# ponimatkin/freepose

Hardware: AMD Instinct MI355X
Metric: proposals/sec (ViT-L feat + top-k + 576-pose render-compare) (higher is better)
Workload: dtype bf16

## Files before the change

freepose_amd/csrc/capi.hip:

```cpp
#include <stdarg.h>
#include <stdio.h>

#include "../../include/freepose_hip.h"
#include "tower_steps.h"
#include "pnp_core.h"
#include "video_eval_core.h"
#include "gt_info_core.h"
#include "lk_core.h"

static thread_local char g_err[512] = "";
void fp_set_error(const char* fmt, ...) {
    va_list ap;
    va_start(ap, fmt);
    vsnprintf(g_err, sizeof(g_err), fmt, ap);
    va_end(ap);
}
extern "C" const char* fp_last_error(void) { return g_err; }
extern "C" int fp_version(void) { return 100; }

#ifdef FP_LAB
static int g_opts[FP_OPT_COUNT] = {-1, -1, -1, -1, -1, -1, -1, -1, -1, -1, -1, -1};
int fp_opt_get(int key, int dflt) { return (key >= 0 && key < FP_OPT_COUNT && g_opts[key] >= 0) ? g_opts[key] : dflt; }
extern "C" int fp_lab_set_option(const char* name, int value) {
    FP_REQUIRE(name, "lab_set_option: null name");
// ... 544 lines not shown
    return fp_attention_hd_fwd((const bf16_t*)QKV, ldqkv, (bf16_t*)O, ldo, B, heads, head_dim, n_tok, npad, scale, (hipStream_t)stream);
}
extern "C" int fp_op_attention_causal(const void* QKV, int ldqkv, void* O, int ldo, int B, int heads, int head_dim, int n_tok, int npad,
                                      float scale, void* stream) {
    return fp_attention_causal_fwd((const bf16_t*)QKV, ldqkv, (bf16_t*)O, ldo, B, heads, head_dim, n_tok, npad, scale, (hipStream_t)stream);
}
extern "C" int fp_knn_l2(fp_ctx* ctx, const float* d_table, int N, int E, const float* d_queries, int Q, int k, int32_t* d_out_idx,
                         float* d_out_d2, void* stream) {
    FP_REQUIRE(ctx, "knn_l2: null context");
    FP_REQUIRE(N > 0 && Q > 0, "knn_l2: bad shape N=%d Q=%d", N, Q);
    float* ws = nullptr;
    FP_WS(ctx, "knn.d2", (size_t)Q * N * sizeof(float), ws);
    return fp_knn_l2_launch(d_table, N, E, d_queries, Q, k, ws, d_out_idx, d_out_d2, (hipStream_t)stream);
}
extern "C" int fp_op_im2col_norm(const void* img, void* A, int B, int H, int W, int ps, int KP, void* stream) {
    FP_REQUIRE(img && A && B > 0, "op_im2col_norm: null argument / empty batch");
    return fp_im2col_norm_ms((const bf16_t*)img, (bf16_t*)A, B, H, W, ps, KP, FP_IMAGENET_MEAN, FP_IMAGENET_SD, (hipStream_t)stream);
}
extern "C" int fp_op_layernorm(const void* X, void* Y, const void* g, const void* b, int rows, int D, float eps,
                               void* stream) {
    if (rows == 0) return FP_OK;
    FP_REQUIRE(X && Y && g && b, "op_layernorm: null argument");
    return fp_layernorm((const bf16_t*)X, (bf16_t*)Y, (const bf16_t*)g, (const bf16_t*)b, rows, D, eps, 0, 0, 0,
                        (hipStream_t)stream);
}
extern "C" int fp_op_layernorm_rows(const void* X, void* Y, const void* g, const void* b, int rows, int D, float eps, int rows_per_b,
                                    int in_stride_b, int in_off, int l2_normalize, void* stream) {
    FP_REQUIRE(rows >= 0 && D >= 0, "op_layernorm_rows: rows=%d, D=%d", rows, D);
    if (rows == 0 || D == 0) return FP_OK;
    FP_REQUIRE(X && Y && g && b, "op_layernorm_rows: null argument");
    FP_REQUIRE(rows_per_b <= 0 || (in_stride_b >= 0 && in_off >= 0), "op_layernorm_rows: in_stride_b=%d, in_off=%d (>= 0)", in_stride_b, in_off);
    return fp_layernorm((const bf16_t*)X, (bf16_t*)Y, (const bf16_t*)g, (const bf16_t*)b, rows, D, eps, rows_per_b, in_stride_b, in_off,
                        (hipStream_t)stream, l2_normalize != 0);
}
extern "C" int fp_op_posembed_aa(const void* src, void* dst, int G, int gh, int gw, int D, void* stream) {
    FP_REQUIRE(G >= 0 && gh >= 0 && gw >= 0 && D >= 0, "op_posembed_aa: G=%d, gh=%d, gw=%d, D=%d", G, gh, gw, D);
    if (gh == 0 || gw == 0 || D == 0) return FP_OK;
    FP_REQUIRE(src && dst, "op_posembed_aa: null argument");
    return fp_posembed_aa((const bf16_t*)src, (bf16_t*)dst, G, gh, gw, D, (hipStream_t)stream);
}
extern "C" int fp_op_token_init(void* X, const void* cls, const void* pos0, const void* reg, int nreg, int B, int n_tok, int npad, int D,
                                void* stream) {
    FP_REQUIRE(B >= 0 && B <= 65535 && D >= 0, "op_token_init: B=%d (0..65535), D=%d", B, D);
    FP_REQUIRE(nreg >= 0 && n_tok >= 1 + nreg && npad >= n_tok, "op_token_init: nreg=%d, n_tok=%d, npad=%d (1 + nreg <= n_tok <= npad)", nreg, n_tok,
               npad);
    if (B == 0 || D == 0) return FP_OK;
    FP_REQUIRE(X && cls && pos0 && (reg || nreg == 0), "op_token_init: null argument");
    FP_REQUIRE((long long)(1 + nreg + npad - n_tok) * D <= INT32_MAX, "op_token_init: %d rows of %d elements", 1 + nreg + npad - n_tok, D);
    return fp_token_init((bf16_t*)X, (const bf16_t*)cls, (const bf16_t*)pos0, (const bf16_t*)reg, nreg, B, n_tok, npad, D, (hipStream_t)stream);
}
extern "C" int fp_op_row_stats(const void* X, int rows, int D, float eps, void* d_rec, float* d_rstd, void* stream) {
    FP_REQUIRE(rows >= 0 && D >= 0, "op_row_stats: rows=%d, D=%d", rows, D);
    if (rows == 0) return FP_OK;
    FP_REQUIRE(X && d_rec && d_rstd, "op_row_stats: null argument");
    FP_REQUIRE(D > 0, "op_row_stats: D=%d", D);
    return fp_row_stats((const bf16_t*)X, (uint4*)d_rec, d_rstd, rows, D, eps, (hipStream_t)stream);
}
extern "C" int fp_op_stats_finalize(const void* part, int rows, int D, float eps, int part_ld, void* d_rec, float* d_rstd, void* stream) {
    FP_REQUIRE(rows >= 0 && D >= 0, "op_stats_finalize: rows=%d, D=%d", rows, D);
    if (rows == 0) return FP_OK;
    FP_REQUIRE(part && d_rec && d_rstd, "op_stats_finalize: null argument");
    FP_REQUIRE(D > 0 && (part_ld == 0 || part_ld >= rows), "op_stats_finalize: D=%d, part_ld=%d (0 or >= rows=%d)", D, part_ld, rows);
    return fp_stats_finalize((const float2*)part, (uint4*)d_rec, d_rstd, rows, D, eps, (hipStream_t)stream, part_ld);
}
extern "C" int fp_op_ln_fold(const void* W, const void* gamma, const void* beta, const void* bias, int N, int K, int n_scaled, float row_scale,
                             void* Wf, void* d_cb, void* stream) {
    FP_REQUIRE(N >= 0 && K >= 0, "op_ln_fold: N=%d, K=%d", N, K);
    if (N == 0) return FP_OK;
    FP_REQUIRE(K > 0 && n_scaled >= 0 && n_scaled <= N, "op_ln_fold: K=%d, n_scaled=%d outside [0, N=%d]", K, n_scaled, N);
    return fp_ln_fold((const bf16_t*)W, (const bf16_t*)gamma, (const bf16_t*)beta, (const bf16_t*)bias, (bf16_t*)Wf, (uint4*)d_cb, N, K, n_scaled,
                      row_scale, (hipStream_t)stream);
}
extern "C" int fp_op_transpose(const void* src, void* dst, int rows, int cols, void* stream) {
    FP_REQUIRE(rows >= 0 && cols >= 0, "op_transpose: rows=%d, cols=%d", rows, cols);
    if (rows == 0 || cols == 0) return FP_OK;
    FP_REQUIRE(src && dst, "op_transpose: null argument");
    return fp_transpose_bf16((const bf16_t*)src, (bf16_t*)dst, rows, cols, (hipStream_t)stream);
}

struct FpTimer { hipEvent_t a, b; };
extern "C" int fp_timer_create(void** out) {
    FP_REQUIRE(out, "timer_create: null");
    FpTimer* t = new FpTimer();
    FP_HIP(hipEventCreate(&t->a));
    FP_HIP(hipEventCreate(&t->b));
    *out = t;
    return FP_OK;
}
extern "C" int fp_timer_start(void* t, void* s) { FP_HIP(hipEventRecord(((FpTimer*)t)->a, (hipStream_t)s)); return FP_OK; }
extern "C" int fp_timer_stop(void* t, void* s) { FP_HIP(hipEventRecord(((FpTimer*)t)->b, (hipStream_t)s)); return FP_OK; }
extern "C" int fp_timer_elapsed_ms(void* t, float* ms) {
    FP_HIP(hipEventSynchronize(((FpTimer*)t)->b));
    FP_HIP(hipEventElapsedTime(ms, ((FpTimer*)t)->a, ((FpTimer*)t)->b));
    return FP_OK;
}
extern "C" int fp_timer_destroy(void* t) {
    if (!t) return FP_OK;
    (void)hipEventDestroy(((FpTimer*)t)->a);
    (void)hipEventDestroy(((FpTimer*)t)->b);
    delete (FpTimer*)t;
    return FP_OK;
}

#define FP_LK_MAX_QUERIES (1 << 20)
static int lk_check_sizes(const char* what, int T, int H, int W, int levels, int radius) {
    FP_REQUIRE(T >= 1 && T <= 65535, "%s: T=%d frames (1..65535)", what, T);
    FP_REQUIRE(H >= 1 && W >= 1 && H <= FP_LK_MAX_SIDE && W <= FP_LK_MAX_SIDE, "%s: %d x %d frames (1..%d per side)", what, H, W, FP_LK_MAX_SIDE);
    FP_REQUIRE((long long)T * H * W <= (1ll << 30), "%s: T * H * W = %lld pixels (at most 2^30 per call)", what, (long long)T * H * W);
    FP_REQUIRE(radius >= 1 && radius <= FP_LK_MAX_RADIUS, "%s: radius=%d (1..%d)", what, radius, FP_LK_MAX_RADIUS);
    FP_REQUIRE(levels >= 1 && levels <= FP_LK_MAX_LEVELS, "%s: levels=%d (1..%d)", what, levels, FP_LK_MAX_LEVELS);
    return FP_OK;
}

extern "C" int fp_lk_pyramid(fp_ctx* ctx, const uint8_t* d_frames, int T, int H, int W, int levels, int radius, float* d_pyramid, void* stream) {
    FP_REQUIRE(ctx && d_frames && d_pyramid, "lk_pyramid: null argument");
    if (int rc = lk_check_sizes("lk_pyramid", T, H, W, levels, radius)) return rc;
    LkPyramid P;
    lk_pyramid_layout(T, H, W, levels, radius, P);
    return fp_lk_pyramid_launch(d_frames, P, d_pyramid, (hipStream_t)stream);
}

extern "C" int fp_lk_track(fp_ctx* ctx, const float* d_pyramid, int T, int H, int W, int levels, const float* d_queries, int N, int radius,
                           int iters, float fb_thresh, float min_eig, float max_residual, float* d_tracks, uint8_t* d_vis, float* d_diag,
                           void* stream) {
    if (int rc = lk_check_sizes("lk_track", T, H, W, levels, radius)) return rc;
    FP_REQUIRE(N >= 0 && N <= FP_LK_MAX_QUERIES, "lk_track: N=%d queries (0..2^20)", N);
    FP_REQUIRE(ctx && d_pyramid && (N == 0 || (d_queries && d_tracks && d_vis && d_diag)), "lk_track: null argument");
    FP_REQUIRE(iters >= 1 && iters <= FP_LK_MAX_ITERS, "lk_track: iters=%d (1..%d)", iters, FP_LK_MAX_ITERS);
    LkPyramid P;
    lk_pyramid_layout(T, H, W, levels, radius, P);
    double* state = nullptr;
    if (N > 0) FP_WS(ctx, "lk_state", (size_t)T * N * 2 * sizeof(double), state);
    return fp_lk_track_launch(P, d_pyramid, d_queries, N, radius, iters, fb_thresh, min_eig, max_residual, state, d_tracks, d_vis, d_diag,
                              (hipStream_t)stream);
}
```

freepose_amd/csrc/tower_steps.h:

```cpp
#pragma once
#include <stdio.h>
#include <string.h>

#include <cmath>

#include "internal.h"

struct GemmStep {
    FpGemmArgs g{};
    int epi;
    GemmStep(const bf16_t* X, int ldx, const bf16_t* W, int K, bf16_t* C, int ldc, const bf16_t* bias, int M, int N, bool gelu = false)
        : epi(gelu ? FP_EPI_BIAS_GELU : FP_EPI_BIAS) {
        g.X = X; g.ldx = ldx; g.W = W; g.ldw = K; g.C = C; g.ldc = ldc; g.bias = bias;
        g.M = M; g.N = N; g.K = K;
    }
    GemmStep& residual(const bf16_t* gamma, const bf16_t* resid, int ldr, float2* stat_part = nullptr) {
        g.gamma = gamma; g.resid = resid; g.ldr = ldr; g.stat_part = stat_part;
        epi = stat_part ? FP_EPI_LS_RES_STATS : FP_EPI_BIAS_LS_RES;
        return *this;
    }
    GemmStep& transposed_v(int npad, int heads) {
        g.ldc = 8; g.npad = npad; g.heads = heads;
        epi = FP_EPI_VT;
        return *this;
    }
    GemmStep& patch_embed(const bf16_t* pos, int P, int npad, int tok_off) {
        g.pos = pos; g.P = P; g.npad = npad; g.tok_off = tok_off;
        epi = FP_EPI_PATCH;
        return *this;
    }
    int run(fp_ctx* ctx, hipStream_t s) { return ctx->gemm(g, epi, s); }
};

struct LnStats {
    uint4* stat; float* rstd; float2* part;
    int M, D; float eps;
    bool pending = false;
    int ready(const bf16_t* rows, int N, hipStream_t s) {
        pending = !rows && fp_gemm_fuses_ln_part(M, N);
        if (rows) return fp_row_stats(rows, stat, rstd, M, D, eps, s);
        return pending ? FP_OK : fp_stats_finalize(part, stat, rstd, M, D, eps, s);
    }
    int attach(GemmStep& t, const uint4* cfrag) {
        FP_REQUIRE(t.epi == FP_EPI_BIAS || t.epi == FP_EPI_BIAS_GELU || t.epi == FP_EPI_VT, "ln attach: epilogue %d has no LN-folded form", t.epi);
        t.g.ln_mfrag = stat; t.g.ln_rstd = rstd; t.g.ln_cfrag = cfrag;
        t.epi = t.epi == FP_EPI_BIAS ? FP_EPI_LN_BIAS : (t.epi == FP_EPI_BIAS_GELU ? FP_EPI_LN_GELU : FP_EPI_LN_VT);
        if (pending) { t.g.ln_part = part; t.g.ln_part_ld = M; t.g.ln_part_nb = D / 64; t.g.ln_eps = eps; t.g.ln_inv_d = 1.0f / (float)D; }
        pending = false;
        return FP_OK;
    }
};

enum TowerCls { TOWER_GEMM = 0, TOWER_ATTN = 1, TOWER_OTHER = 2 };
struct TowerProf {
    bool on = false;
    struct EvPair { hipEvent_t a, b; int cls; };
    std::vector<EvPair> ev_pool;
    size_t ev_used = 0;
    double gemm_flops = 0;
    long gemm_launches = 0;
    void count(double flops, int launches) { if (on) { gemm_flops += flops; gemm_launches += launches; } }
};
struct ProfScope {
    TowerProf* p; hipStream_t s; size_t slot;
    ProfScope(TowerProf* p_, hipStream_t s_, TowerCls cls) : p(p_), s(s_), slot((size_t)-1) {
        if (!p || !p->on) return;
        if (p->ev_used == p->ev_pool.size()) {
            TowerProf::EvPair e{};
            if (hipEventCreate(&e.a) != hipSuccess || hipEventCreate(&e.b) != hipSuccess) return;
            p->ev_pool.push_back(e);
        }
        slot = p->ev_used++;
        p->ev_pool[slot].cls = cls;
        (void)hipEventRecord(p->ev_pool[slot].a, s);
    }
    ~ProfScope() {
        if (slot != (size_t)-1) (void)hipEventRecord(p->ev_pool[slot].b, s);
    }
};

struct TowerBlockW {
    const bf16_t *n1w = nullptr, *n1b = nullptr, *qkvw = nullptr, *qkvb = nullptr, *projw = nullptr,
                 *projb = nullptr, *ls1 = nullptr, *n2w = nullptr, *n2b = nullptr, *fc1w = nullptr, *fc1b = nullptr,
                 *fc2w = nullptr, *fc2b = nullptr, *ls2 = nullptr;
    bool complete() const { return n1w && n1b && qkvw && qkvb && projw && projb && n2w && n2b && fc1w && fc1b && fc2w && fc2b; }
};
struct TowerRun {
    fp_ctx* ctx; TowerProf* prof; hipStream_t s;
    int B, n_tok, npad, D, mlp_dim;
    float eps;
    bf16_t *R, *T, *AO, *H1;
    const bf16_t* ones;
    int M() const { return B * npad; }
    void count(double flops_per_row, int launches) const { if (prof) prof->count((double)B * n_tok * flops_per_row, launches); }
};
struct TowerEmbedW {
    int patch = 0, KP = 0, n_reg = 0;
    const float *mean = nullptr, *sd = nullptr;
    bf16_t* pe_w = nullptr;
    const bf16_t *pe_b = nullptr, *cls = nullptr, *pos = nullptr, *reg = nullptr;
};
inline int fp_tower_embed(const TowerRun& t, const TowerEmbedW& e, const bf16_t* pos_patch, const bf16_t* img, int H, int W, bf16_t* A0, bf16_t* X) {
    const int P = (H / e.patch) * (W / e.patch);
    int rc;
    {
        ProfScope ps(t.prof, t.s, TOWER_OTHER);
        if ((rc = fp_im2col_norm_ms(img, A0, t.B, H, W, e.patch, e.KP, e.mean, e.sd, t.s))) return rc;
        if ((rc = fp_token_init(X, e.cls, e.pos, e.reg, e.n_reg, t.B, t.n_tok, t.npad, t.D, t.s))) return rc;
    }
    ProfScope ps(t.prof, t.s, TOWER_GEMM);
    GemmStep pe(A0, e.KP, e.pe_w, e.KP, X, t.D, e.pe_b, t.B * P, t.D);
    if ((rc = pe.patch_embed(pos_patch, P, t.npad, 1 + e.n_reg).run(t.ctx, t.s))) return rc;
    if (t.prof) t.prof->count(2.0 * t.B * P * (3.0 * e.patch * e.patch) * t.D, 1);
    return FP_OK;
}
inline int fp_tower_out_proj(const TowerRun& t, const TowerBlockW& w, float2* stat_part) {
    ProfScope ps(t.prof, t.s, TOWER_GEMM);
    GemmStep proj(t.AO, t.D, w.projw, t.D, t.R, t.D, w.projb, t.M(), t.D);
    if (int rc = proj.residual(w.ls1 ? w.ls1 : t.ones, t.R, t.D, stat_part).run(t.ctx, t.s)) return rc;
    t.count(2.0 * t.D * t.D, 1);
    return FP_OK;
}
inline int fp_tower_mlp(const TowerRun& t, const TowerBlockW& w, LnStats* st, const bf16_t* fc1w, const uint4* fc1_cb, float2* stat_part) {
    const int D = t.D, M = t.M(), N = t.mlp_dim;
    int rc;
    {
        ProfScope ps(t.prof, t.s, TOWER_OTHER);
        if ((rc = st ? st->ready(nullptr, N, t.s) : fp_layernorm(t.R, t.T, w.n2w, w.n2b, M, D, t.eps, 0, 0, 0, t.s))) return rc;
    }
    ProfScope ps(t.prof, t.s, TOWER_GEMM);
    GemmStep fc1(st ? t.R : t.T, D, st ? fc1w : w.fc1w, D, t.H1, N, w.fc1b, M, N, true);
    if (st && (rc = st->attach(fc1, fc1_cb))) return rc;
    if ((rc = fc1.run(t.ctx, t.s))) return rc;
    if ((rc = GemmStep(t.H1, N, w.fc2w, N, t.R, D, w.fc2b, M, D).residual(w.ls2 ? w.ls2 : t.ones, t.R, D, stat_part).run(t.ctx, t.s))) return rc;
    t.count(4.0 * D * N, 2);
    return FP_OK;
}

inline bool fp_weight_numel(const char* who, const char* name, size_t numel, size_t want) {
    if (numel != want) fp_set_error("%s: %s has %zu elements, expected %zu", who, name, numel, want);
    return numel == want;
}
struct WeightEnt { const char* n; const bf16_t** slot; size_t numel; };
template <size_t N>
inline int fp_set_named_weight(const char* who, const char* name, const char* rest, const WeightEnt (&tab)[N], const bf16_t* p, size_t numel) {
    for (const WeightEnt& e : tab)
        if (!strcmp(rest, e.n)) {
            if (!fp_weight_numel(who, name, numel, e.numel)) return -1;
            *e.slot = p;
            return 1;
        }
    return 0;
}
inline int fp_tower_set_patch_weight(const char* who, const char* name, const bf16_t* p, size_t numel, const TowerEmbedW& e, size_t D, hipStream_t s) {
    const size_t K = (size_t)3 * e.patch * e.patch;
    if (!fp_weight_numel(who, name, numel, D * K)) return FP_ERR_INVALID;
    FP_HIP(hipMemcpy2DAsync(e.pe_w, (size_t)e.KP * 2, p, K * 2, K * 2, D, hipMemcpyDeviceToDevice, s));
    return FP_OK;
}

// ... 84 lines not shown
```

freepose_amd/csrc/vit.hip:

```cpp
#include <stdio.h>

#include "../../include/freepose_hip.h"
#include "tower_steps.h"

struct fp_vit {
    fp_ctx* ctx = nullptr;
    fp_vit_arch a{};
    TowerEmbedW emb;
    const bf16_t *normw = nullptr, *normb = nullptr;
    bf16_t* ones = nullptr;
    std::vector<TowerBlockW> blk;
    struct VitFold { bf16_t *qkvw = nullptr, *fc1w = nullptr; uint4 *qkv_cb = nullptr, *fc1_cb = nullptr; };
    std::vector<VitFold> fold;
    int folded_upto = 0;
    hipEvent_t fold_ev = nullptr;
    hipStream_t fold_stream = nullptr;
    bool refold = false;
    std::map<std::pair<int, int>, bf16_t*> pos_cache;
    TowerProf prof;
};

extern "C" int fp_vit_create(fp_ctx* ctx, const fp_vit_arch* arch, fp_vit** out) {
    FP_REQUIRE(ctx && arch && out, "vit_create: null argument");
    FP_REQUIRE(arch->dim % 64 == 0 && arch->heads * 64 == arch->dim, "vit_create: dim=%d heads=%d (head dim must be 64)",
               arch->dim, arch->heads);
    FP_REQUIRE(arch->mlp_dim % 64 == 0 && arch->depth > 0 && arch->patch > 0, "vit_create: bad arch");
    fp_vit* v = new fp_vit();
    v->ctx = ctx;
    v->a = *arch;
    v->blk.resize(arch->depth);
    v->fold.resize(arch->depth);
    v->emb.patch = arch->patch; v->emb.n_reg = arch->n_reg; v->emb.mean = FP_IMAGENET_MEAN; v->emb.sd = FP_IMAGENET_SD;
    v->emb.KP = cdiv(3 * arch->patch * arch->patch, 64) * 64;
    if (hipMalloc((void**)&v->emb.pe_w, (size_t)arch->dim * v->emb.KP * 2) != hipSuccess ||
        hipMalloc((void**)&v->ones, (size_t)arch->dim * 2) != hipSuccess) {
        fp_set_error("vit_create: hipMalloc failed");
        delete v;
        return FP_ERR_HIP;
    }
    FP_HIP(hipMemset(v->emb.pe_w, 0, (size_t)arch->dim * v->emb.KP * 2));
    std::vector<bf16_t> one(arch->dim, f2bf(1.0f));
    FP_HIP(hipMemcpy(v->ones, one.data(), (size_t)arch->dim * 2, hipMemcpyHostToDevice));
    *out = v;
    return FP_OK;
}
extern "C" int fp_vit_destroy(fp_vit* v) {
    if (!v) return FP_OK;
    if (v->emb.pe_w) (void)hipFree(v->emb.pe_w);
    if (v->ones) (void)hipFree(v->ones);
    for (auto& kv : v->pos_cache) (void)hipFree(kv.second);
    for (auto& f : v->fold) {
        if (f.qkvw) (void)hipFree(f.qkvw);
        if (f.fc1w) (void)hipFree(f.fc1w);
        if (f.qkv_cb) (void)hipFree(f.qkv_cb);
        if (f.fc1_cb) (void)hipFree(f.fc1_cb);
    }
    for (auto& p : v->prof.ev_pool) { (void)hipEventDestroy(p.a); (void)hipEventDestroy(p.b); }
    if (v->fold_ev) (void)hipEventDestroy(v->fold_ev);
    delete v;
    return FP_OK;
}

extern "C" int fp_vit_set_weight(fp_vit* v, const char* name, const void* d, size_t numel, void* stream) {
    FP_REQUIRE(v && name && d, "vit_set_weight: null argument");
    const fp_vit_arch& a = v->a;
    const bf16_t* p = (const bf16_t*)d;
    const size_t D = a.dim;
    if (v->folded_upto > 0) v->refold = true;
    v->folded_upto = 0;
    std::string s(name);
    if (s == "pos_embed") {
        if (!fp_weight_numel("vit_set_weight", name, numel, (size_t)(1 + a.pos_grid * a.pos_grid) * D)) return FP_ERR_INVALID;
        v->emb.pos = p;
        for (auto& kv : v->pos_cache) (void)hipFree(kv.second);
        v->pos_cache.clear();
        return FP_OK;
    }
    if (s == "mask_token") return FP_OK;
    if (s == "patch_embed.proj.weight") return fp_tower_set_patch_weight("vit_set_weight", name, p, numel, v->emb, D, (hipStream_t)stream);
    const WeightEnt top[] = {{"cls_token", &v->emb.cls, D}, {"register_tokens", &v->emb.reg, (size_t)a.n_reg * D}, {"patch_embed.proj.bias", &v->emb.pe_b, D},
                             {"norm.weight", &v->normw, D}, {"norm.bias", &v->normb, D}};
    if (const int hit = fp_set_named_weight("vit_set_weight", name, name, top, p, numel)) return hit > 0 ? FP_OK : FP_ERR_INVALID;
    int bi = -1;
    char rest[64] = {0};
    if (sscanf(name, "blocks.%d.%63s", &bi, rest) == 2 && bi >= 0 && bi < a.depth) {
        TowerBlockW& w = v->blk[bi];
        const size_t M = a.mlp_dim;
        const WeightEnt tab[] = {
            {"norm1.weight", &w.n1w, D}, {"norm1.bias", &w.n1b, D},
            {"attn.qkv.weight", &w.qkvw, 3 * D * D}, {"attn.qkv.bias", &w.qkvb, 3 * D},
            {"attn.proj.weight", &w.projw, D * D}, {"attn.proj.bias", &w.projb, D},
            {"ls1.gamma", &w.ls1, D}, {"norm2.weight", &w.n2w, D}, {"norm2.bias", &w.n2b, D},
            {"mlp.fc1.weight", &w.fc1w, M * D}, {"mlp.fc1.bias", &w.fc1b, M},
            {"mlp.fc2.weight", &w.fc2w, D * M}, {"mlp.fc2.bias", &w.fc2b, D}, {"ls2.gamma", &w.ls2, D}};
        if (const int hit = fp_set_named_weight("vit_set_weight", name, rest, tab, p, numel)) return hit > 0 ? FP_OK : FP_ERR_INVALID;
    }
    fp_set_error("vit_set_weight: unknown tensor name '%s'", name);
    return FP_ERR_INVALID;
}

static int vit_pos(fp_vit* v, int gh, int gw, hipStream_t s, const bf16_t** out) {
    const fp_vit_arch& a = v->a;
    if (gh == a.pos_grid && gw == a.pos_grid) { *out = v->emb.pos + a.dim; return FP_OK; }
    auto key = std::make_pair(gh, gw);
    auto it = v->pos_cache.find(key);
    if (it == v->pos_cache.end()) {
        bf16_t* buf = nullptr;
        FP_HIP(hipMalloc((void**)&buf, (size_t)gh * gw * a.dim * 2));
        int rc = fp_posembed_aa(v->emb.pos + a.dim, buf, a.pos_grid, gh, gw, a.dim, s);
        if (rc) { (void)hipFree(buf); return rc; }
        it = v->pos_cache.emplace(key, buf).first;
    }
    *out = it->second;
    return FP_OK;
}

static int vit_fold(fp_vit* v, int first, int L, hipStream_t s) {
    const fp_vit_arch& a = v->a;
    const size_t D = a.dim, Mm = a.mlp_dim;
    for (int i = first; i < L; ++i) {
        const TowerBlockW& w = v->blk[i];
        fp_vit::VitFold& f = v->fold[i];
        if (!f.qkvw) FP_HIP(hipMalloc((void**)&f.qkvw, 3 * D * D * 2));
        if (!f.qkv_cb) FP_HIP(hipMalloc((void**)&f.qkv_cb, 3 * D * sizeof(uint4)));
        if (!f.fc1w) FP_HIP(hipMalloc((void**)&f.fc1w, Mm * D * 2));
        if (!f.fc1_cb) FP_HIP(hipMalloc((void**)&f.fc1_cb, Mm * sizeof(uint4)));
        int rc;
        if ((rc = fp_ln_fold(w.qkvw, w.n1w, w.n1b, w.qkvb, f.qkvw, f.qkv_cb, (int)(3 * D), (int)D, (int)D, FP_ATTN_QSCALE, s))) return rc;
        if ((rc = fp_ln_fold(w.fc1w, w.n2w, w.n2b, w.fc1b, f.fc1w, f.fc1_cb, (int)Mm, (int)D, 0, 1.0f, s))) return rc;
    }
    return FP_OK;
}

extern "C" double fp_vit_flops(const fp_vit* v, int B, int H, int W, int layer) {
    const fp_vit_arch& a = v->a;
    const double P = (double)(H / a.patch) * (W / a.patch), N = P + 1 + a.n_reg, D = a.dim;
    const int L = std::min(layer, a.depth);
    const double mlp_ratio = (double)a.mlp_dim / a.dim;
    const double per_block = (8.0 + 4.0 * mlp_ratio) * N * D * D + 4.0 * N * N * D;
    return B * (L * per_block + 2.0 * P * (3.0 * a.patch * a.patch) * D);
}

extern "C" int fp_vit_forward(fp_vit* v, const void* d_images, int B, int H, int W, int layer, int feature_type,
                              void* d_out, void* stream) {
    FP_REQUIRE(v && d_images && d_out, "vit_forward: null argument");
    const fp_vit_arch& a = v->a;
    hipStream_t s = (hipStream_t)stream;
    fp_ctx* ctx = v->ctx;
    FP_REQUIRE(B > 0 && H % a.patch == 0 && W % a.patch == 0, "vit_forward: B=%d H=%d W=%d (patch %d)", B, H, W, a.patch);
    FP_REQUIRE(feature_type >= 0 && feature_type <= 3, "vit_forward: feature_type %d", feature_type);
    FP_REQUIRE(v->emb.cls && v->emb.pos && v->emb.pe_b && v->normw && v->normb && (a.n_reg == 0 || v->emb.reg),
               "vit_forward: embedding / final-norm weights not set");
    const int L = (layer >= 1 && layer <= a.depth) ? layer : a.depth;
    for (int i = 0; i < L; ++i) {
        FP_REQUIRE(v->blk[i].complete(), "vit_forward: weights of block %d not set", i);
    }
    const int D = a.dim, gh = H / a.patch, gw = W / a.patch, P = gh * gw;
    const int n_tok = P + 1 + a.n_reg;
    const int npad = cdiv(n_tok, 16) * 16;
    const size_t M = (size_t)B * npad;
    FP_REQUIRE(M * (size_t)a.mlp_dim * 2 < 0xffffffffull, "vit_forward: batch too large for 32-bit tile offsets (B=%d)", B);
    const int Mi = (int)M;

    bf16_t *A0, *X, *Y, *QK, *Vt, *AO, *H1;
    int rc;
    const bool lnf = ctx->opt_ln_fused != 0 && D % 64 == 0;
    LnStats st{nullptr, nullptr, nullptr, Mi, D, a.ln_eps};
    if (lnf) {
        if (v->fold_ev && s != v->fold_stream) FP_HIP(hipStreamWaitEvent(s, v->fold_ev, 0));
        if (v->folded_upto < L) {
            if (v->refold) {
                FP_HIP(hipDeviceSynchronize());
                v->refold = false;
            }
            if ((rc = vit_fold(v, v->folded_upto, L, s))) return rc;
            if (!v->fold_ev) FP_HIP(hipEventCreateWithFlags(&v->fold_ev, hipEventDisableTiming));
            FP_HIP(hipEventRecord(v->fold_ev, s));
            v->fold_stream = s;
            v->folded_upto = L;
        }
        FP_WS(ctx, "vit.ln_stat", M * sizeof(uint4), st.stat);
        FP_WS(ctx, "vit.ln_rstd", M * sizeof(float), st.rstd);
        FP_WS(ctx, "vit.ln_part", M * (size_t)(D / 64) * sizeof(float2), st.part);
    }
    FP_WS(ctx, "vit.im2col", (size_t)B * P * v->emb.KP * 2, A0);
    FP_WS(ctx, "vit.x", M * D * 2, X);
    FP_WS(ctx, "vit.y", M * D * 2, Y);
    FP_WS(ctx, "vit.qk", M * 2 * D * 2, QK);
    FP_WS(ctx, "vit.vt", M * D * 2 + 256, Vt);
    FP_WS(ctx, "vit.ao", M * D * 2, AO);
    FP_WS(ctx, "vit.h1", M * (size_t)a.mlp_dim * 2, H1);

    const bf16_t* pos_patch;
    if ((rc = vit_pos(v, gh, gw, s, &pos_patch))) return rc;

    const TowerRun t{ctx, &v->prof, s, B, n_tok, npad, D, a.mlp_dim, a.ln_eps, X, Y, AO, H1, v->ones};
    if ((rc = fp_tower_embed(t, v->emb, pos_patch, (const bf16_t*)d_images, H, W, A0, X))) return rc;
    const bf16_t* in = lnf ? X : Y;
    for (int i = 0; i < L; ++i) {
        const TowerBlockW& w = v->blk[i];
        const fp_vit::VitFold& f = v->fold[i];
        {
            ProfScope ps(&v->prof, s, TOWER_OTHER);
            if ((rc = lnf ? st.ready(i == 0 ? X : nullptr, 2 * D, s) : fp_layernorm(X, Y, w.n1w, w.n1b, Mi, D, a.ln_eps, 0, 0, 0, s))) return rc;
        }
        {
            ProfScope ps(&v->prof, s, TOWER_GEMM);
            const bf16_t* qkvw = lnf ? f.qkvw : w.qkvw;
            GemmStep qk(in, D, qkvw, D, QK, 2 * D, w.qkvb, Mi, 2 * D), vt(in, D, qkvw + (size_t)2 * D * D, D, Vt, 8, w.qkvb + 2 * D, Mi, D);
            vt.transposed_v(npad, a.heads);
            if (lnf && ((rc = st.attach(qk, f.qkv_cb)) || (rc = st.attach(vt, f.qkv_cb + 2 * D)))) return rc;
            if ((rc = qk.run(ctx, s))) return rc;
            if ((rc = vt.run(ctx, s))) return rc;
            t.count(2.0 * 3.0 * D * D, 2);
        }
        {
            ProfScope ps(&v->prof, s, TOWER_ATTN);
            if ((rc = fp_attention_fwd(QK, 2 * D, Vt, AO, D, B, a.heads, n_tok, npad, lnf, s))) return rc;
        }
        if ((rc = fp_tower_out_proj(t, w, st.part))) return rc;
        if ((rc = fp_tower_mlp(t, w, lnf ? &st : nullptr, f.fc1w, f.fc1_cb, i + 1 < L ? st.part : nullptr))) return rc;
    }
    {
        ProfScope ps(&v->prof, s, TOWER_OTHER);
        const int rows_per_b = feature_type == 0 ? 1 : (feature_type == 1 ? a.n_reg : P);
        const int off = feature_type == 0 ? 0 : (feature_type == 1 ? 1 : 1 + a.n_reg);
        if (rows_per_b > 0)
            if ((rc = fp_layernorm(X, (bf16_t*)d_out, v->normw, v->normb, B * rows_per_b, D, a.ln_eps, rows_per_b, npad,
                                   off, s, feature_type == 3)))
                return rc;
    }
    return FP_OK;
}

extern "C" int fp_vit_profile(fp_vit* v, int enable) {
    FP_REQUIRE(v, "vit_profile: null");
    TowerProf& p = v->prof;
    p.on = enable != 0;
    p.ev_used = 0;
    p.gemm_flops = 0;
    p.gemm_launches = 0;
    return FP_OK;
}
extern "C" int fp_vit_profile_read(fp_vit* v, float* g, float* at, float* o, double* fl) {
    FP_REQUIRE(v, "vit_profile_read: null");
    TowerProf& p = v->prof;
    float acc[3] = {0.f, 0.f, 0.f};
    for (size_t i = 0; i < p.ev_used; ++i) {
        FP_HIP(hipEventSynchronize(p.ev_pool[i].b));
        float ms = 0.f;
        FP_HIP(hipEventElapsedTime(&ms, p.ev_pool[i].a, p.ev_pool[i].b));
        acc[p.ev_pool[i].cls] += ms;
    }
    if (g) *g = acc[TOWER_GEMM];
    if (at) *at = acc[TOWER_ATTN];
    if (o) *o = acc[TOWER_OTHER];
    if (fl) *fl = p.gemm_flops;
    return FP_OK;
}
extern "C" long fp_vit_profile_gemm_launches(const fp_vit* v) { return v ? v->prof.gemm_launches : 0; }
```

freepose_amd/csrc/vit_misc.hip:

```cpp
#include "internal.h"
#include "dot64.h"
#include "gemm_bf16.h"

namespace {

__global__ void im2col_norm_kernel(const bf16_t* __restrict__ img, bf16_t* __restrict__ A, int B, int H,
                                   int W, int ps, int KP, float m0, float m1, float m2, float s0, float s1,
                                   float s2) {
    const int gw = W / ps, gh = H / ps, P = gw * gh;
    const int K = 3 * ps * ps;
    const int chunks = KP / 8;
    const long total = (long)B * P * chunks;
    for (long idx = blockIdx.x * (long)blockDim.x + threadIdx.x; idx < total;
         idx += (long)gridDim.x * blockDim.x) {
        const int ch = (int)(idx % chunks);
        const long row = idx / chunks;
        const int b = (int)(row / P), pp = (int)(row % P);
        const int py = pp / gw, px = pp % gw;
        uint32_t w[4];
#pragma unroll
        for (int e = 0; e < 8; e += 2) {
            float v[2];
#pragma unroll
            for (int u = 0; u < 2; ++u) {
                const int k = ch * 8 + e + u;
                float val = 0.f;
                if (k < K) {
                    const int c = k / (ps * ps), rem = k % (ps * ps);
                    const int dy = rem / ps, dx = rem % ps;
                    const float x = bf2f(img[(((size_t)b * 3 + c) * H + (py * ps + dy)) * W + px * ps + dx]);
                    const float mean = c == 0 ? m0 : (c == 1 ? m1 : m2);
                    const float sd = c == 0 ? s0 : (c == 1 ? s1 : s2);
                    val = rbf(rbf(x - mean) / sd);
                }
                v[u] = val;
            }
            w[e / 2] = pack_bf2(v[0], v[1]);
        }
        *(uint4*)(A + (size_t)row * KP + ch * 8) = make_uint4(w[0], w[1], w[2], w[3]);
    }
}

__global__ void token_init_kernel(bf16_t* __restrict__ X, const bf16_t* __restrict__ cls,
                                  const bf16_t* __restrict__ pos0, const bf16_t* __restrict__ reg, int nreg,
                                  int n_tok, int npad, int D) {
    const int b = blockIdx.y;
    const int nrows = 1 + nreg + (npad - n_tok);
    for (int i = blockIdx.x * blockDim.x + threadIdx.x; i < nrows * D; i += gridDim.x * blockDim.x) {
        const int r = i / D, c = i % D;
        int row;
        bf16_t v;
        if (r == 0) { row = 0; v = f2bf(bf2f(cls[c]) + bf2f(pos0[c])); }
        else if (r <= nreg) { row = r; v = reg[(r - 1) * D + c]; }
        else { row = n_tok + (r - 1 - nreg); v = 0; }
        X[((size_t)b * npad + row) * D + c] = v;
    }
}

template <int MAXC, int L2 = 0>
__global__ __launch_bounds__(256) void layernorm_kernel(const bf16_t* __restrict__ X, bf16_t* __restrict__ Y,
                                                        const bf16_t* __restrict__ gamma,
                                                        const bf16_t* __restrict__ beta, int rows, int D,
                                                        float eps, int rows_per_b, int in_stride_b, int in_off) {
    const int lane = threadIdx.x & 63;
    const int wave = (blockIdx.x * blockDim.x + threadIdx.x) >> 6;
    const int nwave = (gridDim.x * blockDim.x) >> 6;
    const int nch = D / 8;
    for (int r = wave; r < rows; r += nwave) {
        const size_t ir = (size_t)(r / rows_per_b) * in_stride_b + in_off + (r % rows_per_b);
        const bf16_t* xr = X + ir * D;
        uint4 xw[MAXC];
        float v[MAXC][8];
        d64_load<MAXC>(xw, xr, 0, D, lane);
        d64_unpack(xw, v);
        float sum = 0.f;
#pragma unroll
        for (int c = 0; c < MAXC; ++c)
            if (lane + 64 * c < nch) {
#pragma unroll
                for (int e = 0; e < 8; ++e) sum += v[c][e];
            }
        const float mean = wave_sum(sum) / (float)D;
        float sq = 0.f;
#pragma unroll
        for (int c = 0; c < MAXC; ++c)
            if (lane + 64 * c < nch) {
#pragma unroll
                for (int e = 0; e < 8; ++e) { const float d = v[c][e] - mean; sq += d * d; }
            }
        const float rstd = rsqrtf(wave_sum(sq) / (float)D + eps);
        bf16_t* yr = Y + (size_t)r * D;
        uint4 keep[MAXC];
        float acc = 0.f;
#pragma unroll
        for (int c = 0; c < MAXC; ++c) {
            const int ch = lane + 64 * c;
            if (ch < nch) {
                const uint4 g = *(const uint4*)(gamma + ch * 8), bb = *(const uint4*)(beta + ch * 8);
                const uint32_t gw[4] = {g.x, g.y, g.z, g.w}, bw[4] = {bb.x, bb.y, bb.z, bb.w};
                uint32_t o[4];
#pragma unroll
                for (int e = 0; e < 4; ++e) {
                    const float a = (v[c][2 * e] - mean) * rstd * lo_bf(gw[e]) + lo_bf(bw[e]);
                    const float b = (v[c][2 * e + 1] - mean) * rstd * hi_bf(gw[e]) + hi_bf(bw[e]);
                    o[e] = pack_bf2(a, b);
                }
                if (L2) {
                    keep[c] = make_uint4(o[0], o[1], o[2], o[3]);
                    acc = d64_sumsq(keep[c], acc);
                } else {
                    *(uint4*)(yr + ch * 8) = make_uint4(o[0], o[1], o[2], o[3]);
                }
            }
        }
        if (L2) d64_norm_store<MAXC>(keep, d64_row_norm(wave_sum(acc)), yr, D, lane);
    }
}

__device__ __forceinline__ float cubic_aa(float x) {
    const float a = -0.5f;
    x = fabsf(x);
    if (x < 1.f) return ((a + 2.f) * x - (a + 3.f)) * x * x + 1.f;
// ... 203 lines not shown
            }
        const float sigma = __fsqrt_rn(wave_sum(sq) / (float)D + eps);
        if (lane == 0) { mfrag[r] = ln_row_record(mean, sigma); rstd_out[r] = __builtin_amdgcn_rcpf(sigma); }

    }
}

__global__ __launch_bounds__(256) void stats_finalize_kernel(const float2* __restrict__ part, uint4* __restrict__ mfrag,
                                                             float* __restrict__ rstd_out, int rows, int nb, float inv_d, float eps, int part_ld) {
    const int r = blockIdx.x * blockDim.x + threadIdx.x;
    if (r >= rows) return;
    uint4 rec;
    float rstd;
    fp_ln_finalize_row(part, (size_t)part_ld, nb, r, inv_d, eps, rec, rstd);
    mfrag[r] = rec;
    rstd_out[r] = rstd;
}

__global__ __launch_bounds__(256) void ln_fold_kernel(const bf16_t* __restrict__ W, const bf16_t* __restrict__ gamma,
                                                      const bf16_t* __restrict__ beta, const bf16_t* __restrict__ bias,
                                                      bf16_t* __restrict__ Wf, uint4* __restrict__ cfrag, int N, int K, int n_scaled,
                                                      float row_scale) {
    const int lane = threadIdx.x & 63;
    const int n = (blockIdx.x * blockDim.x + threadIdx.x) >> 6;
    if (n >= N) return;
    const float rs = n < n_scaled ? row_scale : 1.0f;
    float cs = 0.f, wb = 0.f;
    for (int k = lane * 8; k < K; k += 512) {
        const uint4 w = *(const uint4*)(W + (size_t)n * K + k), g = *(const uint4*)(gamma + k), b = *(const uint4*)(beta + k);
        const uint32_t ww[4] = {w.x, w.y, w.z, w.w}, gw[4] = {g.x, g.y, g.z, g.w}, bw[4] = {b.x, b.y, b.z, b.w};
        uint32_t o[4];
#pragma unroll
        for (int e = 0; e < 4; ++e) {
            const float f0 = rbf(lo_bf(ww[e]) * lo_bf(gw[e]) * rs), f1 = rbf(hi_bf(ww[e]) * hi_bf(gw[e]) * rs);
            o[e] = pack_bf2(f0, f1);
            cs += f0;
            cs += f1;
            wb = __fmaf_rn(lo_bf(ww[e]), lo_bf(bw[e]), wb);
            wb = __fmaf_rn(hi_bf(ww[e]), hi_bf(bw[e]), wb);
        }
        *(uint4*)(Wf + (size_t)n * K + k) = make_uint4(o[0], o[1], o[2], o[3]);
    }
    cs = wave_sum(cs);
    wb = wave_sum(wb);
    if (lane == 0) {
        const float bp = ((bias ? bf2f(bias[n]) : 0.f) + wb) * rs;
        const float bh = rbf(bp), bl = rbf(bp - bh), ch = rbf(cs), cl = rbf(cs - ch);
        cfrag[n] = make_uint4(pack_bf2(bh, bh), pack_bf2(bl, ch), pack_bf2(ch, cl), 0u);
    }
}

}

int fp_row_stats(const bf16_t* X, uint4* ms, float* rstd, int rows, int D, float eps, hipStream_t s) {
    FP_REQUIRE(D % 8 == 0 && D <= 8 * 64 * 3, "row_stats: D=%d unsupported", D);
    if (rows <= 0) return FP_OK;
    const int blocks = std::min(cdiv(rows, 4), 256 * 8);
    if (D <= 512) hipLaunchKernelGGL(row_stats_kernel<1>, dim3(blocks), dim3(256), 0, s, X, ms, rstd, rows, D, eps);
    else if (D <= 1024) hipLaunchKernelGGL(row_stats_kernel<2>, dim3(blocks), dim3(256), 0, s, X, ms, rstd, rows, D, eps);
    else hipLaunchKernelGGL(row_stats_kernel<3>, dim3(blocks), dim3(256), 0, s, X, ms, rstd, rows, D, eps);
    FP_LAUNCH_CHECK();
    return FP_OK;
}

int fp_stats_finalize(const float2* part, uint4* ms, float* rstd, int rows, int D, float eps, hipStream_t s, int part_ld) {
    FP_REQUIRE(D % 64 == 0, "stats_finalize: D=%d must be a multiple of 64", D);
    if (rows <= 0) return FP_OK;
    hipLaunchKernelGGL(stats_finalize_kernel, dim3(cdiv(rows, 256)), dim3(256), 0, s, part, ms, rstd, rows, D / 64, 1.0f / (float)D, eps, part_ld > 0 ? part_ld : rows);
    FP_LAUNCH_CHECK();
    return FP_OK;
}

int fp_ln_fold(const bf16_t* W, const bf16_t* gamma, const bf16_t* beta, const bf16_t* bias, bf16_t* Wf, uint4* cb, int N, int K,
               int n_scaled, float row_scale, hipStream_t s) {
    FP_REQUIRE(W && gamma && beta && bias && Wf && cb, "ln_fold: null argument (W / LayerNorm gamma, beta / bias / outputs)");
    FP_REQUIRE(N > 0 && K % 8 == 0, "ln_fold: N=%d, K=%d (K must be a multiple of 8)", N, K);
    hipLaunchKernelGGL(ln_fold_kernel, dim3(cdiv(N, 4)), dim3(256), 0, s, W, gamma, beta, bias, Wf, cb, N, K, n_scaled, row_scale);
    FP_LAUNCH_CHECK();
    return FP_OK;
}

int fp_im2col_norm_ms(const bf16_t* img, bf16_t* A, int B, int H, int W, int ps, int KP, const float* mean, const float* sd, hipStream_t s) {
    FP_REQUIRE(H % ps == 0 && W % ps == 0 && KP % 8 == 0 && KP >= 3 * ps * ps, "im2col: bad shape");
    const long total = (long)B * (H / ps) * (W / ps) * (KP / 8);
    const int blocks = (int)std::min<long>((total + 255) / 256, 256 * 16);
    hipLaunchKernelGGL(im2col_norm_kernel, dim3(blocks), dim3(256), 0, s, img, A, B, H, W, ps, KP, rbf(mean[0]), rbf(mean[1]), rbf(mean[2]),
                       rbf(sd[0]), rbf(sd[1]), rbf(sd[2]));
    FP_LAUNCH_CHECK();
    return FP_OK;
}

int fp_token_init(bf16_t* X, const bf16_t* cls, const bf16_t* pos0, const bf16_t* reg, int nreg, int B,
                  int n_tok, int npad, int D, hipStream_t s) {
    const int nrows = 1 + nreg + (npad - n_tok);
    if (B <= 0 || D <= 0) return FP_OK;
    hipLaunchKernelGGL(token_init_kernel, dim3(cdiv(nrows * D, 256), B), dim3(256), 0, s, X, cls, pos0, reg, nreg,
                       n_tok, npad, D);
    FP_LAUNCH_CHECK();
    return FP_OK;
}

int fp_layernorm(const bf16_t* X, bf16_t* Y, const bf16_t* gamma, const bf16_t* beta, int rows, int D, float eps,
                 int rows_per_b, int in_stride_b, int in_off, hipStream_t s, int l2_normalize) {
    FP_REQUIRE(D % 8 == 0 && D <= 8 * 64 * 4, "layernorm: D=%d unsupported", D);
    FP_REQUIRE(!l2_normalize || D <= 8 * 64 * 3, "layernorm: D=%d with l2_normalize unsupported", D);
    if (rows <= 0) return FP_OK;
    if (rows_per_b <= 0) { rows_per_b = rows; in_stride_b = 0; in_off = 0; }
    const int blocks = std::min(cdiv(rows, 4), 256 * 8);
#define FP_LN(C, L) hipLaunchKernelGGL((layernorm_kernel<C, L>), dim3(blocks), dim3(256), 0, s, X, Y, gamma, beta, rows, D, eps, rows_per_b, in_stride_b, in_off)
    if (D <= 512) { if (l2_normalize) FP_LN(1, 1); else FP_LN(1, 0); }
    else if (D <= 1024) { if (l2_normalize) FP_LN(2, 1); else FP_LN(2, 0); }
    else if (D <= 1536) { if (l2_normalize) FP_LN(3, 1); else FP_LN(3, 0); }
    else FP_LN(4, 0);
#undef FP_LN
    FP_LAUNCH_CHECK();
    return FP_OK;
}

int fp_posembed_aa(const bf16_t* src, bf16_t* dst, int G, int gh, int gw, int D, hipStream_t s) {
    FP_REQUIRE(G > 0 && gh > 0 && gw > 0, "posembed: bad grid");
    FP_REQUIRE(4.0f * G / gh + 2 < AA_MAX_TAPS && 4.0f * G / gw + 2 < AA_MAX_TAPS, "posembed: downscale factor too large (grid %d -> %d x %d)", G, gh, gw);
    hipLaunchKernelGGL(posembed_aa_kernel, dim3(gh * gw), dim3(256), 0, s, src, dst, G, gh, gw, D);
    FP_LAUNCH_CHECK();
    return FP_OK;
}

int fp_ffa_pool(const bf16_t* feats, const uint8_t* mask, bf16_t* out, float* out_f32, int B, int P, int D, int gh,
                int gw, int cell, uint8_t* pm_scratch, hipStream_t s, bf16_t* out_norm, int* arrive) {
    FP_REQUIRE(gh * gw == P && D % 2 == 0 && cell >= 1, "ffa: bad shape P=%d gh=%d gw=%d", P, gh, gw);
    FP_REQUIRE(P <= 60000 && cell * cell * gw <= 60000, "ffa: P=%d cell=%d too large for the LDS staging", P, cell);
    const uint8_t* pm = mask;
    if (cell > 1) {
        FP_REQUIRE(pm_scratch, "ffa: no patch-mask scratch");
        hipLaunchKernelGGL(ffa_cellmask_kernel, dim3(gh, B), dim3(256), (size_t)cell * cell * gw, s, mask, pm_scratch, gh, gw, cell);
        FP_LAUNCH_CHECK();
        pm = pm_scratch;
    }
    FP_REQUIRE(!arrive || (out && out_norm && D % 8 == 0), "ffa: the fused normalisation needs both bf16 buffers and D %% 8 == 0");
    hipLaunchKernelGGL(ffa_kernel, dim3(cdiv(D, 64), B), dim3(1024), P, s, feats, pm, out, out_f32, P, D, out_norm, arrive);
    FP_LAUNCH_CHECK();
    return FP_OK;
}

int fp_transpose_bf16(const bf16_t* src, bf16_t* dst, int rows, int cols, hipStream_t s) {
    const size_t total = (size_t)rows * cols;
    if (total == 0) return FP_OK;
    hipLaunchKernelGGL(transpose_bf16_kernel, dim3((unsigned)std::min<size_t>((total + 255) / 256, 4096)), dim3(256), 0, s, src, dst, rows, cols);
    FP_LAUNCH_CHECK();
    return FP_OK;
}

int fp_l2norm_rows(const bf16_t* X, bf16_t* Y, int rows, int D, hipStream_t s) {
    FP_REQUIRE(D % 8 == 0, "l2norm: D must be a multiple of 8");
    if (rows == 0) return FP_OK;
    const int nch = cdiv(D, 512);
    const bool aligned = (((uintptr_t)X | (uintptr_t)Y) & 15) == 0;
    if (nch <= 3 && aligned) {
        fp_nch_dispatch(nch, [&](auto c) {
            hipLaunchKernelGGL(l2norm_rows_vec_kernel<decltype(c)::value>, dim3(cdiv(rows, 4)), dim3(256), 0, s, X, Y, rows, D);
        });
    } else
    hipLaunchKernelGGL(l2norm_rows_kernel, dim3(rows), dim3(64), 0, s, X, Y, rows, D);
    FP_LAUNCH_CHECK();
    return FP_OK;
}
```

Before: 1.982.

## Stage im2col patch strips through LDS and lighten profiling events

Adds an im2col kernel that reads coalesced image rows for a strip of patches, normalizes them into a padded LDS tile, then writes full patch rows with 16-byte stores. It falls back to the old gather kernel when shapes do not fit. This targets the uncoalesced per-element gather in patch embedding. Separately, profiling and timer events are created without the system fence, and consecutive profile scopes share boundary events so fewer events are recorded.

New measurement: 1.995 (median of 6 runs). Within noise of the previous version (+0.6%).

```diff
diff --git a/freepose_amd/csrc/capi.hip b/freepose_amd/csrc/capi.hip
--- a/freepose_amd/csrc/capi.hip
+++ b/freepose_amd/csrc/capi.hip
@@ -650,8 +650,8 @@
 extern "C" int fp_timer_create(void** out) {
     FP_REQUIRE(out, "timer_create: null");
     FpTimer* t = new FpTimer();
-    FP_HIP(hipEventCreate(&t->a));
-    FP_HIP(hipEventCreate(&t->b));
+    FP_HIP(fp_stopwatch_event(&t->a));
+    FP_HIP(fp_stopwatch_event(&t->b));
     *out = t;
     return FP_OK;
 }
diff --git a/freepose_amd/csrc/tower_steps.h b/freepose_amd/csrc/tower_steps.h
--- a/freepose_amd/csrc/tower_steps.h
+++ b/freepose_amd/csrc/tower_steps.h
@@ -52,30 +52,50 @@
 };
 
 enum TowerCls { TOWER_GEMM = 0, TOWER_ATTN = 1, TOWER_OTHER = 2 };
+inline hipError_t fp_stopwatch_event(hipEvent_t* ev) { return hipEventCreateWithFlags(ev, hipEventDisableSystemFence); }
 struct TowerProf {
+    static constexpr size_t NONE = (size_t)-1;
     bool on = false;
-    struct EvPair { hipEvent_t a, b; int cls; };
-    std::vector<EvPair> ev_pool;
+    std::vector<hipEvent_t> ev_pool;
     size_t ev_used = 0;
+    struct Span { size_t a, b; int cls; };
+    std::vector<Span> spans;
+    size_t chain = NONE;
+    hipStream_t chain_stream = nullptr;
     double gemm_flops = 0;
     long gemm_launches = 0;
     void count(double flops, int launches) { if (on) { gemm_flops += flops; gemm_launches += launches; } }
+    void reset() { ev_used = 0; spans.clear(); chain = NONE; gemm_flops = 0; gemm_launches = 0; }
+    void break_chain() { chain = NONE; }
+    size_t mark(hipStream_t s) {
+        if (ev_used == ev_pool.size()) {
+            hipEvent_t e;
+            if (fp_stopwatch_event(&e) != hipSuccess) return NONE;
+            ev_pool.push_back(e);
+        }
+        if (hipEventRecord(ev_pool[ev_used], s) != hipSuccess) return NONE;
+        return ev_used++;
+    }
+    void destroy() {
+        for (hipEvent_t e : ev_pool) (void)hipEventDestroy(e);
+        ev_pool.clear();
+        reset();
+    }
 };
 struct ProfScope {
-    TowerProf* p; hipStream_t s; size_t slot;
-    ProfScope(TowerProf* p_, hipStream_t s_, TowerCls cls) : p(p_), s(s_), slot((size_t)-1) {
+    TowerProf* p; hipStream_t s; size_t a; int cls;
+    ProfScope(TowerProf* p_, hipStream_t s_, TowerCls cls_) : p(p_), s(s_), a(TowerProf::NONE), cls(cls_) {
         if (!p || !p->on) return;
-        if (p->ev_used == p->ev_pool.size()) {
-            TowerProf::EvPair e{};
-            if (hipEventCreate(&e.a) != hipSuccess || hipEventCreate(&e.b) != hipSuccess) return;
-            p->ev_pool.push_back(e);
-        }
-        slot = p->ev_used++;
-        p->ev_pool[slot].cls = cls;
-        (void)hipEventRecord(p->ev_pool[slot].a, s);
+        a = (p->chain != TowerProf::NONE && p->chain_stream == s) ? p->chain : p->mark(s);
+        p->chain = TowerProf::NONE;
     }
     ~ProfScope() {
-        if (slot != (size_t)-1) (void)hipEventRecord(p->ev_pool[slot].b, s);
+        if (a == TowerProf::NONE) return;
+        const size_t b = p->mark(s);
+        if (b == TowerProf::NONE) return;
+        p->spans.push_back({a, b, cls});
+        p->chain = b;
+        p->chain_stream = s;
     }
 };
 
diff --git a/freepose_amd/csrc/vit.hip b/freepose_amd/csrc/vit.hip
--- a/freepose_amd/csrc/vit.hip
+++ b/freepose_amd/csrc/vit.hip
@@ -55,7 +55,7 @@
         if (f.qkv_cb) (void)hipFree(f.qkv_cb);
         if (f.fc1_cb) (void)hipFree(f.fc1_cb);
     }
-    for (auto& p : v->prof.ev_pool) { (void)hipEventDestroy(p.a); (void)hipEventDestroy(p.b); }
+    v->prof.destroy();
     if (v->fold_ev) (void)hipEventDestroy(v->fold_ev);
     delete v;
     return FP_OK;
@@ -195,6 +195,7 @@
     if ((rc = vit_pos(v, gh, gw, s, &pos_patch))) return rc;
 
     const TowerRun t{ctx, &v->prof, s, B, n_tok, npad, D, a.mlp_dim, a.ln_eps, X, Y, AO, H1, v->ones};
+    v->prof.break_chain();
     if ((rc = fp_tower_embed(t, v->emb, pos_patch, (const bf16_t*)d_images, H, W, A0, X))) return rc;
     const bf16_t* in = lnf ? X : Y;
     for (int i = 0; i < L; ++i) {
@@ -237,20 +238,18 @@
     FP_REQUIRE(v, "vit_profile: null");
     TowerProf& p = v->prof;
     p.on = enable != 0;
-    p.ev_used = 0;
-    p.gemm_flops = 0;
-    p.gemm_launches = 0;
+    p.reset();
     return FP_OK;
 }
 extern "C" int fp_vit_profile_read(fp_vit* v, float* g, float* at, float* o, double* fl) {
     FP_REQUIRE(v, "vit_profile_read: null");
     TowerProf& p = v->prof;
     float acc[3] = {0.f, 0.f, 0.f};
-    for (size_t i = 0; i < p.ev_used; ++i) {
-        FP_HIP(hipEventSynchronize(p.ev_pool[i].b));
+    for (const TowerProf::Span& sp : p.spans) {
+        FP_HIP(hipEventSynchronize(p.ev_pool[sp.b]));
         float ms = 0.f;
-        FP_HIP(hipEventElapsedTime(&ms, p.ev_pool[i].a, p.ev_pool[i].b));
-        acc[p.ev_pool[i].cls] += ms;
+        FP_HIP(hipEventElapsedTime(&ms, p.ev_pool[sp.a], p.ev_pool[sp.b]));
+        acc[sp.cls] += ms;
     }
     if (g) *g = acc[TOWER_GEMM];
     if (at) *at = acc[TOWER_ATTN];
diff --git a/freepose_amd/csrc/vit_misc.hip b/freepose_amd/csrc/vit_misc.hip
--- a/freepose_amd/csrc/vit_misc.hip
+++ b/freepose_amd/csrc/vit_misc.hip
@@ -38,6 +38,77 @@
             w[e / 2] = pack_bf2(v[0], v[1]);
         }
         *(uint4*)(A + (size_t)row * KP + ch * 8) = make_uint4(w[0], w[1], w[2], w[3]);
+    }
+}
+
+constexpr int IM2COL_LDS_PAD = 16;
+constexpr int IM2COL_UNROLL = 8;
+constexpr int IM2COL_THREADS = 256;
+constexpr int IM2COL_UNITS = 128;
+
+template <int VEC>
+__global__ __launch_bounds__(IM2COL_THREADS) void im2col_strip_kernel(const bf16_t* __restrict__ img, bf16_t* __restrict__ A, int H,
+                                                                      int W, int ps, int KP, int pw, int nseg, float m0, float m1,
+                                                                      float m2, float s0, float s1, float s2) {
+    extern __shared__ uint4 im2col_tile[];
+    bf16_t* tile = (bf16_t*)im2col_tile;
+    const int tid = threadIdx.x;
+    const int gw = W / ps, gh = H / ps;
+    const int LS = KP + IM2COL_LDS_PAD;
+    const int seg = blockIdx.x % nseg, strip = blockIdx.x / nseg;
+    const int py = strip % gh, b = strip / gh;
+    const int px0 = seg * pw, pwa = min(pw, gw - px0);
+    const int K = 3 * ps * ps;
+    const uint32_t HW = (uint32_t)H * W;
+    const bf16_t* src = img + (size_t)b * 3 * HW + (size_t)py * ps * W + (size_t)px0 * ps;
+
+    for (int p = tid >> 6; p < pwa; p += IM2COL_THREADS / 64)
+        for (int k = K + (tid & 63); k < KP; k += 64) tile[p * LS + k] = 0;
+
+    const int nW = pwa * ps / VEC;
+    const int G = IM2COL_THREADS / nW;
+    const int g = tid / nW;
+    if (g < G) {
+        const int x = (tid - g * nW) * VEC, p = x / ps;
+        const int dst0 = p * LS + (x - p * ps);
+        const int spare = pw * LS;
+        const float mean[3] = {m0, m1, m2}, sd[3] = {s0, s1, s2};
+        for (int dy0 = g; dy0 < ps; dy0 += G * IM2COL_UNROLL) {
+            uint32_t v[3][IM2COL_UNROLL];
+#pragma unroll
+            for (int c = 0; c < 3; ++c)
+#pragma unroll
+                for (int j = 0; j < IM2COL_UNROLL; ++j) {
+                    const int dy = dy0 + j * G;
+                    const uint32_t off = (dy < ps ? (uint32_t)dy * W : 0u) + c * HW + x;
+                    v[c][j] = VEC == 2 ? *(const uint32_t*)(src + off) : (uint32_t)src[off];
+                }
+#pragma unroll
+            for (int c = 0; c < 3; ++c)
+#pragma unroll
+                for (int j = 0; j < IM2COL_UNROLL; ++j) {
+                    const int dy = dy0 + j * G;
+                    const int dst = dy < ps ? dst0 + (c * ps + dy) * ps : spare;
+                    if (VEC == 2) {
+                        const float lo = rbf(rbf(lo_bf(v[c][j]) - mean[c]) / sd[c]), hi = rbf(rbf(hi_bf(v[c][j]) - mean[c]) / sd[c]);
+                        *(uint32_t*)(tile + dst) = pack_bf2(lo, hi);
+                    } else {
+                        tile[dst] = f2bf(rbf(bf2f((bf16_t)v[c][j]) - mean[c]) / sd[c]);
+                    }
+                }
+        }
+    }
+    __syncthreads();
+
+    const int n16 = KP / 8, total = pwa * n16;
+    uint4* out = (uint4*)(A + ((size_t)strip * gw + px0) * KP);
+    int pr = tid / n16, c16 = tid - pr * n16;
+    const int dpr = IM2COL_THREADS / n16, dc16 = IM2COL_THREADS - dpr * n16;
+#pragma unroll 4
+    for (int i = tid; i < total; i += IM2COL_THREADS) {
+        out[i] = *(const uint4*)(tile + pr * LS + c16 * 8);
+        pr += dpr; c16 += dc16;
+        if (c16 >= n16) { c16 -= n16; ++pr; }
     }
 }
 
@@ -407,10 +478,26 @@
 
 int fp_im2col_norm_ms(const bf16_t* img, bf16_t* A, int B, int H, int W, int ps, int KP, const float* mean, const float* sd, hipStream_t s) {
     FP_REQUIRE(H % ps == 0 && W % ps == 0 && KP % 8 == 0 && KP >= 3 * ps * ps, "im2col: bad shape");
+    if (B <= 0 || H == 0 || W == 0) return FP_OK;
+    const float m0 = rbf(mean[0]), m1 = rbf(mean[1]), m2 = rbf(mean[2]), s0 = rbf(sd[0]), s1 = rbf(sd[1]), s2 = rbf(sd[2]);
+    const int gw = W / ps, gh = H / ps;
+    const size_t row_bytes = (size_t)(KP + IM2COL_LDS_PAD) * 2;
+    const long strips = (long)B * gh;
+    if (row_bytes <= 48 * 1024 && ps <= IM2COL_THREADS && 3l * H * W < (1l << 31) && strips * gw < (1l << 31)) {
+        const bool pairs = ps % 2 == 0 && ((uintptr_t)img & 3) == 0;
+        const int by_units = IM2COL_UNITS * (pairs ? 2 : 1) / ps, by_lds = (int)(24 * 1024 / row_bytes);
+        const int pw = std::max(1, std::min(gw, std::min(by_units, by_lds)));
+        const int nseg = cdiv(gw, pw);
+        const dim3 grid((unsigned)(strips * nseg));
+#define FP_IM2COL(V) hipLaunchKernelGGL(im2col_strip_kernel<V>, grid, dim3(IM2COL_THREADS), (size_t)pw * row_bytes + 16, s, img, A, H, W, ps, KP, pw, nseg, m0, m1, m2, s0, s1, s2)
+        if (pairs) FP_IM2COL(2); else FP_IM2COL(1);
+#undef FP_IM2COL
+        FP_LAUNCH_CHECK();
+        return FP_OK;
+    }
     const long total = (long)B * (H / ps) * (W / ps) * (KP / 8);
     const int blocks = (int)std::min<long>((total + 255) / 256, 256 * 16);
-    hipLaunchKernelGGL(im2col_norm_kernel, dim3(blocks), dim3(256), 0, s, img, A, B, H, W, ps, KP, rbf(mean[0]), rbf(mean[1]), rbf(mean[2]),
-                       rbf(sd[0]), rbf(sd[1]), rbf(sd[2]));
+    hipLaunchKernelGGL(im2col_norm_kernel, dim3(blocks), dim3(256), 0, s, img, A, B, H, W, ps, KP, m0, m1, m2, s0, s1, s2);
     FP_LAUNCH_CHECK();
     return FP_OK;
 }
```
